# abhro/MonteCarloScattering.jl

Hardware: AMD Instinct MI355X
Metric: particle-scatter steps/sec + wall-time per iter, 10^6 particles, 1->8 MI355X (higher is better)
Workload: dtype f64

## Files before the change

### montecarloscattering.jl_amd/csrc/mcs_api.hip

```cpp
#include "mcs_launch.h"
#include "mcs_hip_owned.h"
#include "mcs_ctx_view.h"
#include "../../include/mcs_ic.h"

#include <cmath>
#include <cstdio>
#include <cstdlib>
#include <cstring>
#include <string>
#include <vector>
#include <chrono>
#include <cstdarg>
#include <memory>
#include <utility>

#define MCS_MEV_ERG_ 1.602176634e-6
namespace {
thread_local std::string g_err;

int fail(const std::string& msg) { g_err = msg; return 1; }
#define HIPCHK(expr)                                                                         \
  do {                                                                                       \
    hipError_t e_ = (expr);                                                                  \
    if (e_ != hipSuccess) return fail(std::string(#expr) + ": " + hipGetErrorString(e_));    \
  } while (0)
#define MCS_ENTER_AS(c, who) do { if (!(c)) return fail(std::string(who) + ": null context"); HIPCHK(hipSetDevice((c)->device)); } while (0)
#define MCS_ENTER(c) MCS_ENTER_AS(c, __func__)

std::string format(const char* f, ...) {
  char b[320];
  va_list ap; va_start(ap, f); std::vsnprintf(b, sizeof b, f, ap); va_end(ap);
  return b;
}
template <class B> int reserve(B& b, long long n) {
  const hipError_t e = b.reserve(n);
  return e == hipSuccess ? 0 : fail(std::string(B::alloc_name()) + ": " + hipGetErrorString(e));
}

constexpr double* DevPop::*kPopF64[8] = {&DevPop::weight, &DevPop::ptot_pf, &DevPop::pb_pf, &DevPop::x_PT_cm,
                                         &DevPop::xn_per, &DevPop::prp_x_cm, &DevPop::acctime_sec, &DevPop::phi_rad};
constexpr double* mcs_soa::*kSoaF64[8] = {&mcs_soa::weight, &mcs_soa::ptot_pf, &mcs_soa::pb_pf, &mcs_soa::x_PT_cm,
                                          &mcs_soa::xn_per, &mcs_soa::prp_x_cm, &mcs_soa::acctime_sec, &mcs_soa::phi_rad};
DevPop pop_view(const PopBuf& b, long long first = 0) {
  DevPop d{};
  for (int i = 0; i < 8; ++i) d.*kPopF64[i] = b.f[i] + first;
  d.meta = b.meta + first;
  return d;
}

struct StragBuf : BufGroup<StragBuf> {
  DevBuf<double> d[2];
  long long cap() const { return d[1].cap() / MCS_STRAG_WORDS; }
  hipError_t grow(long long n) { return reserve_all({n * MCS_STRAG_WORDS, n * MCS_STRAG_WORDS}, d[0], d[1]); }
};
struct FusedBuf : BufGroup<FusedBuf> {
  PinnedBuf<KArgs> h_args; PinnedBuf<PcutDev> h_pd; DevBuf<KArgs> d_args; DevBuf<PcutDev> d_pd;
  long long cap() const { return d_args.cap(); }
  hipError_t grow(long long n) { return reserve_all({n, n + 1, n, n + 1}, h_args, h_pd, d_args, d_pd); }
};

enum Ctr { CTR_WORK, CTR_SAVED, CTR_SCAN, CTR_EXPORT, CTR_MISMATCH, CTR_COUNT = 8 };
enum PipeCtr { PC_WORK, PC_SAVED, PC_SCAN, PC_EXPORT, PC_RES_WORK = PC_EXPORT + 2, PC_RES_SAVED, PC_LATE_WORK, PC_LATE_SAVED, PC_LATE_SCAN, PC_COUNT = 16 };
void set_counters(KArgs& a, unsigned long long* ctr, int work, int saved, int exported) {
  a.work_counter = ctr + work; a.n_saved = ctr + saved; a.strag_count = ctr + exported;
}
}

struct mcs_ctx {
  mcs_params P;
  mcs_layout L;
  int device = 0;
  Stream own_stream;
  hipStream_t stream = nullptr;
  DevBuf<double> d_tab;
  DevBuf<double> d_cuts;
  DevTables tb{};
  std::vector<double> h_inj_fracs, h_pcuts, h_ux;
  DevBuf<double> own_T; DevBuf<unsigned long long> own_I;
  double* d_T = nullptr; unsigned long long* d_I = nullptr;
  PopBuf cur, sav, spare;
  DevBuf<uint8_t> d_lsave;
  long long n = 0;
  long long n_saved_last = 0;
  long long n_run_last = 0;
  long long idx_first = 0, idx_stride = 1;
  const long long* idx_gidx = nullptr;
  bool debug_finals = false;
  int retro_cap = MCS_RETRO_CAP;
  int tail_rounds_last = 0;
  StragBuf strag;
  int64_t opt[MCS_OPT_COUNT] = {};
  long long o(int key) const { return opt[key]; }
  FinalsBuf fin; ScanScratch scan;
  DevBuf<double> d_tally_rep;
  long long rep_n = 0;
  bool rep_dirty = false;
  DevBuf<unsigned long long> d_counters;
  DevBuf<double> d_stage;
  PinnedBuf<KArgs> h_args_pin; DevBuf<KArgs> d_args;
  PinnedBuf<unsigned long long> h_back;
  int i_iter = 1, i_ion = 1;
  double aa = 1, zzq = MCS_QCGS, m = MCS_MP, mc = MCS_MP * MCS_C, pmax_cutoff = 0, density = 1, ewf = 1;
  bool have_grid = false, have_cuts = false;
  bool all_parallel = false;
  int kernel_last = -1;
  FusedBuf fused;
  std::vector<Event> f_ev;
  Stream pp_s2; Event pp_reset;
  Stream pp_s1m, pp_s2m; bool pp_masks_tried = false;
  PopBuf pp_sav2; DevBuf<uint8_t> pp_lsave2; ScanScratch pp_scan;
  DevBuf<unsigned long long> pp_dpc; PinnedBuf<unsigned long long> pp_hpc;
  PinnedBuf<KArgs> pp_hargs; DevBuf<KArgs> pp_dargs; DevBuf<PcutDev> pp_dpdl; PinnedBuf<PcutDev> pp_hpdl;
  int pp_waits_last = 0;
  DevBuf<double> d_ctab, d_cout, d_cscratch; DevBuf<unsigned long long> d_cdiag;
  bool have_cout_dndp = false, have_cout_thermo = false;
  DevBuf<double> d_c2d; bool have_c2d = false;
  int blocks = 0, threads = 256;
  Event ev0, ev1;
  Event acc_ev;
  double last_ms = 0.0;
  int n_cu = 256;
};

namespace {

int ensure_capacity(mcs_ctx* c, long long n) {
  if (n > c->cur.cap() || n > c->sav.cap()) {
    const long long cap = grow_cap(n);
    if (c->n > 0 && c->cur.cap() < cap) {
      PopBuf nb;
      if (reserve(nb, cap)) return 1;
      for (int i = 0; i < 8; ++i) HIPCHK(hipMemcpyAsync(nb.f[i], c->cur.f[i], (size_t)c->n * sizeof(double), hipMemcpyDeviceToDevice, c->stream));
      HIPCHK(hipMemcpyAsync(nb.meta, c->cur.meta, (size_t)c->n * sizeof(uint32_t), hipMemcpyDeviceToDevice, c->stream));
      HIPCHK(hipStreamSynchronize(c->stream));
      c->cur = std::move(nb);
    } else if (reserve(c->cur, cap)) return 1;
    if (reserve(c->sav, cap)) return 1;
  }
  if (n > c->d_lsave.cap() && reserve(c->d_lsave, grow_cap(n))) return 1;
  if (c->debug_finals && n > c->fin.cap() && reserve(c->fin, grow_cap(n))) return 1;
  if (n > c->scan.cap() && reserve(c->scan, grow_cap(n))) return 1;
  return 0;
}

int fill(mcs_ctx* c, long long off, long long n, double v) {
  HIPCHK(mcs_launch_fill(c->d_T + off, n, v, c->stream));
  return 0;
}

int upload_soa(mcs_ctx* c, const PopBuf& b, long long n, const mcs_soa* h) {
  for (int i = 0; i < 8; ++i) HIPCHK(hipMemcpyAsync(b.f[i], h->*kSoaF64[i], (size_t)n * sizeof(double), hipMemcpyHostToDevice, c->stream));
  std::vector<uint32_t> meta((size_t)n);
  for (long long k = 0; k < n; ++k) meta[k] = mcs_pack_meta((int)h->grid[k], (int)h->tcut[k], h->downstream[k] != 0, h->inj[k] != 0);
  HIPCHK(hipMemcpyAsync(b.meta, meta.data(), (size_t)n * sizeof(uint32_t), hipMemcpyHostToDevice, c->stream));
  HIPCHK(hipStreamSynchronize(c->stream));
  return 0;
}
int download_soa(mcs_ctx* c, const PopBuf& b, long long n, mcs_soa* h) {
  for (int i = 0; i < 8; ++i) HIPCHK(hipMemcpyAsync(h->*kSoaF64[i], b.f[i], (size_t)n * sizeof(double), hipMemcpyDeviceToHost, c->stream));
// ... 517 lines not shown
  HIPCHK(mcs_launch_compact(c->d_lsave, n, c->scan.bcounts, c->scan.boffs, c->d_counters + CTR_SCAN, c->scan.src, c->stream));
  HIPCHK(hipMemcpyAsync(c->h_back + CTR_SAVED, c->d_counters + CTR_SAVED, 3 * sizeof(unsigned long long), hipMemcpyDeviceToHost, c->stream));
  HIPCHK(hipStreamSynchronize(c->stream));
  const unsigned long long ns[2] = {c->h_back[CTR_SAVED], c->h_back[CTR_SCAN]};
  if (ws && c->h_back[CTR_EXPORT] != 0) {
    return fail(format("mcs_run_pcut: a bounded wait of the wave-specialised kernel ran out (the launch is incomplete; code 0x%llx)", (unsigned long long)c->h_back[CTR_EXPORT]));
  }
  if (budget == 0) {
    float ms = 0.f;
    HIPCHK(hipEventElapsedTime(&ms, c->ev0, c->ev1));
    ms_total = ms;
  }
  c->last_ms = ms_total;
  c->n_saved_last = (long long)ns[0];
  c->n_run_last = n; c->idx_first = i_prt_offset; c->idx_stride = i_prt_stride; c->idx_gidx = (const long long*)dev_gidx;
  if (ns[0] != ns[1]) return fail("mcs_run_pcut: the kernel's n_saved counter and the count of l_save flags differ");
  if (n_saved) *n_saved = (int64_t)ns[0];
  return 0;
}
int mcs_run_pcut_strided(mcs_ctx* c, int i_pcut, int64_t i_prt_offset, int64_t i_prt_stride, int64_t* n_saved) {
  return run_pcut_impl(c, i_pcut, i_prt_offset, i_prt_stride, nullptr, n_saved);
}
int mcs_run_pcut(mcs_ctx* c, int i_pcut, int64_t i_prt_offset, int64_t* n_saved) { return run_pcut_impl(c, i_pcut, i_prt_offset, 1, nullptr, n_saved); }
int mcs_run_pcut_indexed(mcs_ctx* c, int i_pcut, const int64_t* dev_gidx, int64_t* n_saved) {
  MCS_ENTER(c);
  if (!dev_gidx && c->n > 0) return fail("mcs_run_pcut_indexed: null index list");
  return run_pcut_impl(c, i_pcut, 0, 1, dev_gidx, n_saved);
}

struct PcutOut { int64_t *n_use, *n_saved, *i_mult; double* kernel_ms; int64_t* strag; };

static int species_loop_open(mcs_ctx* c, const char* who, int i_pcut_first, int i_pcut_last, const int64_t* n_target, const PcutOut& o, long long* cap_n) {
  const std::string w = std::string(who) + ": ";
  if (!c->have_grid || !c->have_cuts) return fail(w + "grid/cuts not set");
  if (i_pcut_first < 1 || i_pcut_last > c->tb.n_pcuts || i_pcut_last < i_pcut_first) return fail(w + "pcut range");
  if (!n_target || !o.n_use || !o.n_saved || !o.i_mult) return fail(w + "null argument");
  if (c->o(MCS_OPT_TAIL_BUDGET) > 0 || c->blocks > 0) return fail(w + "not with sliced launches or an explicit launch geometry");
  *cap_n = c->n;
  for (int k = 0; k <= i_pcut_last - i_pcut_first; ++k) { if (n_target[k] < 1) return fail(w + "n_target < 1"); if (n_target[k] > *cap_n) *cap_n = n_target[k]; }
  return ensure_capacity(c, *cap_n) || reserve(c->spare, grow_cap(*cap_n));
}

int mcs_run_pcuts_fused(mcs_ctx* c, int i_pcut_first, int i_pcut_last, const int64_t* n_target, int64_t* n_use_out, int64_t* n_saved_out,
                        int64_t* i_mult_out, double* kernel_ms_out) {
  MCS_ENTER(c);
  const PcutOut o{n_use_out, n_saved_out, i_mult_out, kernel_ms_out, nullptr};
  const int npc = i_pcut_last - i_pcut_first + 1;
  long long cap_n = 0;
  if (species_loop_open(c, "mcs_run_pcuts_fused", i_pcut_first, i_pcut_last, n_target, o, &cap_n)) return 1;
  if (npc > c->fused.cap()) {
    HIPCHK(hipStreamSynchronize(c->stream));
    if (reserve(c->fused, npc)) return 1;
  }
  while ((int)c->f_ev.size() < 2 * npc) { Event e; HIPCHK(e.create()); c->f_ev.push_back(std::move(e)); }
  const DevPop pop[2] = {pop_view(c->cur), pop_view(c->spare)}, sav = pop_view(c->sav);
  for (int k = 0; k < npc; ++k) {
    KArgs& a = c->fused.h_args[k];
    fill_kargs(c, a, i_pcut_first + k, 0, 0, 1, nullptr, 0);
    a.in = pop[k & 1]; a.sv = sav;
    a.n_dev = &c->fused.d_pd[k].n_use;
  }
  const K1Plan k1 = k1_plan(c, cap_n, false, false);
  const int blocks = persistent_grid(cap_n, k1.threads, (long long)c->n_cu * k1.per_cu);
  std::memset(c->fused.h_pd, 0, sizeof(PcutDev) * (size_t)(npc + 1));
  c->fused.h_pd[0].n_use = c->n;
  HIPCHK(hipMemcpyAsync(c->fused.d_args, c->fused.h_args, sizeof(KArgs) * (size_t)npc, hipMemcpyHostToDevice, c->stream));
  HIPCHK(hipMemcpyAsync(c->fused.d_pd, c->fused.h_pd, sizeof(PcutDev) * (size_t)(npc + 1), hipMemcpyHostToDevice, c->stream));
  HIPCHK(hipMemsetAsync(c->d_counters, 0, CTR_COUNT * sizeof(unsigned long long), c->stream));
  const int split_blocks = (int)std::min<long long>((cap_n + 255) / 256, (long long)c->n_cu * 16);
  for (int k = 0; k < npc; ++k) {
    HIPCHK(hipMemsetAsync(c->d_lsave, 0, (size_t)cap_n, c->stream));
    HIPCHK(hipEventRecord(c->f_ev[2 * k], c->stream));
    HIPCHK(mcs_launch_transport(c->fused.d_args + k, k1.kernel, blocks, k1.threads, c->stream));
    HIPCHK(hipEventRecord(c->f_ev[2 * k + 1], c->stream));
    HIPCHK(mcs_launch_finalize_split_dev(c->d_lsave, cap_n, c->scan.bcounts, c->scan.boffs, c->d_counters + CTR_SCAN, c->scan.src, c->fused.d_pd + k, c->fused.d_pd + k + 1,
                                         c->d_counters, (long long)n_target[k], c->d_counters + CTR_MISMATCH, sav, pop[(k + 1) & 1], split_blocks, c->stream));
  }
  c->rep_dirty = true;
  HIPCHK(hipMemcpyAsync(c->fused.h_pd, c->fused.d_pd, sizeof(PcutDev) * (size_t)(npc + 1), hipMemcpyDeviceToHost, c->stream));
  HIPCHK(hipMemcpyAsync(c->h_back + CTR_EXPORT, c->d_counters + CTR_EXPORT, 2 * sizeof(unsigned long long), hipMemcpyDeviceToHost, c->stream));
  HIPCHK(hipStreamSynchronize(c->stream));
  if (c->h_back[CTR_MISMATCH] != 0) return fail("mcs_run_pcuts_fused: the kernel's n_saved counter and the count of l_save flags differ");
  if (is_ws(k1.kernel) && c->h_back[CTR_EXPORT] != 0) return fail("mcs_run_pcuts_fused: a bounded wait of the wave-specialised kernel ran out (a launch is incomplete)");
  double ms_sum = 0.0;
  for (int k = 0; k < npc; ++k) {
    o.n_use[k] = c->fused.h_pd[k].n_use; o.n_saved[k] = c->fused.h_pd[k].n_saved; o.i_mult[k] = c->fused.h_pd[k].i_mult;
    float ms = 0.f;
    HIPCHK(hipEventElapsedTime(&ms, c->f_ev[2 * k], c->f_ev[2 * k + 1]));
    if (o.kernel_ms) o.kernel_ms[k] = ms;
    ms_sum += ms;
  }
  int n_split = 0; while (n_split < npc && c->fused.h_pd[n_split].n_saved > 0) ++n_split;
  if (n_split & 1) std::swap(c->cur, c->spare);
  c->n = c->fused.h_pd[n_split].n_use;
  c->n_run_last = -1; c->n_saved_last = 0;
  c->last_ms = ms_sum; c->tail_rounds_last = npc;
  c->kernel_last = k1.kernel;
  return 0;
}

static int pipelined_pcuts(mcs_ctx* c, const K1Plan& k1, int i_pcut_first, int npc, long long cap_n, const int64_t* n_target,
                           int64_t long_draws, int64_t long_imult_max, const PcutOut& o) {
  unsigned long long* const pc = c->pp_dpc;
  const bool masked = c->pp_s1m && c->pp_s2m;
  hipStream_t s1 = c->stream;
  hipStream_t const s2 = masked ? c->pp_s2m : c->pp_s2;
  hipStream_t const s_alone = masked ? c->stream : c->pp_s2;
  const int side_max = 64;
  const int threads = k1.threads;
  const long long full = (long long)c->n_cu * k1.per_cu;
  const DevPop savb[2] = {pop_view(c->sav), pop_view(c->pp_sav2)};
  uint8_t* lsv[2] = {c->d_lsave, c->pp_lsave2};
  long long nA = c->n, nL = 0;
  long long Bk = long_draws;
  bool side_pending = false;
  int side_blocks = 0;
  long long n1_prev = 0, sofar_prev = 0;
  c->pp_waits_last = 0;
  c->tail_rounds_last = 0;
  c->last_ms = 0.0;
  const bool dbg_pipe = std::getenv("MCS_PIPE_DEBUG") != nullptr;
  for (int k = 0; k < npc; ++k) { o.n_use[k] = 0; o.n_saved[k] = 0; o.i_mult[k] = 1; if (o.kernel_ms) o.kernel_ms[k] = 0.0; if (o.strag) { o.strag[2 * k] = 0; o.strag[2 * k + 1] = 0; } }
  HIPCHK(hipMemsetAsync(pc, 0, PC_COUNT * sizeof(unsigned long long), s1));
  if (nA > 0) HIPCHK(hipMemsetAsync(lsv[0], 0, (size_t)nA, s1));
  auto launch_resume = [&](int i_pcut, int q, long long n_pop, long long n_x, hipStream_t st, bool alone) -> int {
    KArgs& a = c->pp_hargs[1];
    fill_kargs(c, a, i_pcut, n_pop, 0, 1, nullptr, 0);
    a.in = pop_view(c->cur); a.sv = savb[q]; a.l_save = lsv[q];
    set_counters(a, pc, PC_RES_WORK, PC_RES_SAVED, PC_EXPORT + (q ^ 1)); a.strag_out = c->strag.d[q ^ 1];
// ... 498 lines not shown
```

### montecarloscattering.jl_amd/csrc/mcs_launch.h

```cpp
#pragma once
#include "mcs_device.h"

extern "C" {
int mcs_transport_max_entries(void);
hipError_t mcs_launch_transport(const KArgs* a_dev, int kernel, int blocks, int threads, hipStream_t st);
int mcs_transport_ws_threads(void);
hipError_t mcs_launch_finalize_split_dev(const uint8_t* l_save, long long cap_n, unsigned int* block_counts, unsigned long long* block_offsets,
                                         unsigned long long* scan_total, long long* src, PcutDev* pd, PcutDev* pd_next, unsigned long long* counters,
                                         long long n_target, unsigned long long* err, DevPop sv, DevPop out, int split_blocks, hipStream_t st);
hipError_t mcs_launch_compact(const uint8_t* l_save, long long n, unsigned int* block_counts, unsigned long long* block_offsets,
                              unsigned long long* total_dev, long long* src, hipStream_t st);
hipError_t mcs_launch_split(DevPop sv, DevPop out, const long long* src, long long n_new, long long i_mult, hipStream_t st);
hipError_t mcs_launch_compact_match(const uint8_t* l_save, long long n, unsigned int* block_counts, unsigned long long* block_offsets,
                                    unsigned long long* total_dev, long long* src, unsigned int match, hipStream_t st);
hipError_t mcs_launch_late_split(const uint8_t* l_save, long long n, unsigned int* block_counts, unsigned long long* block_offsets,
                                 unsigned long long* total_dev, long long* src, PcutDev* pd, long long i_mult, long long n_main_next, DevPop sv,
                                 DevPop out_at_main_end, int split_blocks, hipStream_t st);
hipError_t mcs_launch_saved_export(DevPop sv, const long long* src, long long n_saved, long long cap, long long first,
                                   long long stride, const long long* gin, long long* gidx, double* f64, uint32_t* meta,
                                   hipStream_t st);
hipError_t mcs_launch_split_import(DevPop out, const double* f64, const uint32_t* meta, long long cap, long long i_mult,
                                   long long first, long long stride, long long n_local, hipStream_t st);
hipError_t mcs_launch_init_pop(DevPop out, const double* ptot_in, const double* weight_in, long long n, long long j_offset,
                               long long j_stride, long long n_total, unsigned long long key, double m, double u, double x_start,
                               int i_grid_start, int relativistic, int fast_push, double xn_per_fine, double x_grid_stop,
                               int n_bins, const double* bin_ptot, const double* bin_weight, const long long* bin_start,
                               hipStream_t st);
hipError_t mcs_launch_fill(double* p, long long n, double v, hipStream_t st);
hipError_t mcs_launch_fold_replicas(double* dst, double* rep, long long n, int n_rep, hipStream_t st);
hipError_t mcs_launch_accumulate_tallies(double* dT, double* sT, unsigned long long* dI, unsigned long long* sI, long long a_lo,
                                         long long a_n, long long b_lo, long long b_n, long long i_lo, long long i_n, hipStream_t st);
hipError_t mcs_launch_copy(double* dst, const double* src, long long n, hipStream_t st);
hipError_t mcs_launch_eval(int fn, long long n, const double* a, const double* b, double* out, hipStream_t st);
hipError_t mcs_launch_eval_hot(int fn, long long n, const double* a, const double* b, double* out, hipStream_t st);
hipError_t mcs_launch_eval_scatter(const KArgs* a_dev, int form, long long n, const double* in, double* out, hipStream_t st);
hipError_t mcs_launch_dndp_cr(const mcs_params* P, const double* psd, const double* gam_sf, const double* ux, const double* tabs,
                              double rest_energy, double n0, double gam0, double* out_dndp, unsigned long long* diag, hipStream_t st);
hipError_t mcs_launch_dndp_2d(const mcs_params* P, const double* psd, const double* therm_sf, const unsigned long long* num_crossings, const double* tabs,
                              double rest_energy, double n0, int therm_from_hist, double gam_x, double beta_x, double* scratch, double* ef, hipStream_t st);
hipError_t mcs_launch_photon_ic(const double* ef, const double* p_edge, const double* field, int n_grid, int NM, int NT, int j_max, int n_nu, int n_photon,
                                double log_min_rm, double bins_per_dec, double mc_e, double beam_area, double* out, hipStream_t st);
hipError_t mcs_launch_photon_pion(const double* dndp_pf, const double* p_edge, const double* target, int n_grid, int NM, int n_photon,
                                  double log_emin_erg, double bins_per_dec, double mc, double aa, double scaling, int i_data, double* out, hipStream_t st);
hipError_t mcs_launch_photon_synch(const double* dndp_pf, const double* p_edge, const double* btot, int n_grid, int NM, int n_photon,
                                   double log_emin_erg, double bins_per_dec, double mc, double* out, hipStream_t st);
hipError_t mcs_launch_thermo(const mcs_params* P, const double* psd, const double* therm_pf, const unsigned long long* num_crossings,
                             const double* gam_sf, const double* ux, const double* tabs, double rest_energy, double mc, double n0,
                             int therm_from_hist, double* scratch, double* out3, hipStream_t st);
}
```

### montecarloscattering.jl_amd/csrc/mcs_population.hip

```cpp
#include "mcs_device.h"
#include "mcs_launch.h"
#include "../../include/mcs_math.h"

#pragma clang fp contract(off)

namespace {
constexpr double TWOPI_ = 6.283185307179586;
constexpr double CC_ = MCS_C;

__device__ __forceinline__ void philox_block(uint32_t c0, uint32_t c1, uint32_t c2, uint32_t c3, uint32_t k0,
                                             uint32_t k1, uint32_t& o0, uint32_t& o1, uint32_t& o2, uint32_t& o3) {
#pragma unroll
  for (int r = 0; r < 10; ++r) {
    const uint32_t hi0 = __umulhi(0xD2511F53u, c0), lo0 = 0xD2511F53u * c0;
    const uint32_t hi1 = __umulhi(0xCD9E8D57u, c2), lo1 = 0xCD9E8D57u * c2;
    const uint32_t n0 = hi1 ^ c1 ^ k0, n2 = hi0 ^ c3 ^ k1;
    c0 = n0; c1 = lo1; c2 = n2; c3 = lo0;
    k0 += 0x9E3779B9u; k1 += 0xBB67AE85u;
  }
  o0 = c0; o1 = c1; o2 = c2; o3 = c3;
}
__device__ __forceinline__ double philox_uniform(unsigned long long key, uint32_t stream, unsigned long long j) {
  const unsigned long long blk = j >> 1;
  uint32_t o0, o1, o2, o3;
// ... 26 lines not shown
  __shared__ unsigned long long sh[1024];
  __shared__ unsigned long long carry;
  if (threadIdx.x == 0) carry = 0;
  __syncthreads();
  for (long long c0 = 0; c0 < nb; c0 += 1024) {
    const long long i = c0 + threadIdx.x;
    const unsigned long long v = i < nb ? counts[i] : 0ull;
    sh[threadIdx.x] = v;
    __syncthreads();
    for (int off = 1; off < 1024; off <<= 1) {
      unsigned long long t = threadIdx.x >= (unsigned)off ? sh[threadIdx.x - off] : 0ull;
      __syncthreads();
      sh[threadIdx.x] += t;
      __syncthreads();
    }
    if (i < nb) offsets[i] = carry + sh[threadIdx.x] - v;
    __syncthreads();
    if (threadIdx.x == 1023) carry += sh[1023];
    __syncthreads();
  }
  if (threadIdx.x == 0) *total = carry;
}

extern "C" __global__ void __launch_bounds__(256)
mcs_k_compact_index(const uint8_t* __restrict__ l_save, long long n, const unsigned long long* __restrict__ offsets,
                    long long* __restrict__ src, unsigned int match) {
  __shared__ unsigned int wcount[4][4];
  const long long base = (long long)blockIdx.x * 1024;
  const int wave = threadIdx.x >> 6, lane = threadIdx.x & 63;
  bool f[4];
  unsigned long long m[4];
#pragma unroll
  for (int r = 0; r < 4; ++r) {
    const long long i = base + r * 256 + threadIdx.x;
    f[r] = i < n && l_save[i] == match;
    m[r] = __ballot(f[r]);
    if (lane == 0) wcount[r][wave] = (unsigned int)__popcll(m[r]);
  }
  __syncthreads();
  unsigned long long run = offsets[blockIdx.x];
#pragma unroll
  for (int r = 0; r < 4; ++r) {
    unsigned long long before = run;
    for (int w = 0; w < wave; ++w) before += wcount[r][w];
    if (f[r]) {
      const unsigned long long rank = before + (unsigned long long)__popcll(m[r] & ((1ull << lane) - 1ull));
      src[rank] = base + r * 256 + threadIdx.x;
    }
    run += wcount[r][0] + wcount[r][1] + wcount[r][2] + wcount[r][3];
  }
}

extern "C" __global__ void __launch_bounds__(256)
mcs_k_count_saved_dev(const uint8_t* __restrict__ l_save, const PcutDev* __restrict__ pd, unsigned int* __restrict__ block_counts) {
  __shared__ unsigned int wsum[4];
  const long long n = pd->n_use;
  const long long base = (long long)blockIdx.x * 1024;
  unsigned int c = 0;
  if (base < n) {
#pragma unroll
    for (int r = 0; r < 4; ++r) {
      const long long i = base + r * 256 + threadIdx.x;
      const bool f = i < n && l_save[i] == 1;
      c += (unsigned int)__popcll(__ballot(f));
    }
  }
  if ((threadIdx.x & 63) == 0) wsum[threadIdx.x >> 6] = c;
  __syncthreads();
  if (threadIdx.x == 0) block_counts[blockIdx.x] = wsum[0] + wsum[1] + wsum[2] + wsum[3];
}
extern "C" __global__ void __launch_bounds__(256)
mcs_k_compact_index_dev(const uint8_t* __restrict__ l_save, const PcutDev* __restrict__ pd, const unsigned long long* __restrict__ offsets,
                        long long* __restrict__ src) {
  __shared__ unsigned int wcount[4][4];
  const long long n = pd->n_use;
  const long long base = (long long)blockIdx.x * 1024;
  if (base >= n) return;
  const int wave = threadIdx.x >> 6, lane = threadIdx.x & 63;
  bool f[4];
  unsigned long long m[4];
#pragma unroll
  for (int r = 0; r < 4; ++r) {
    const long long i = base + r * 256 + threadIdx.x;
    f[r] = i < n && l_save[i] == 1;
    m[r] = __ballot(f[r]);
    if (lane == 0) wcount[r][wave] = (unsigned int)__popcll(m[r]);
  }
  __syncthreads();
  unsigned long long run = offsets[blockIdx.x];
#pragma unroll
  for (int r = 0; r < 4; ++r) {
    unsigned long long before = run;
    for (int w = 0; w < wave; ++w) before += wcount[r][w];
    if (f[r]) {
      const unsigned long long rank = before + (unsigned long long)__popcll(m[r] & ((1ull << lane) - 1ull));
      src[rank] = base + r * 256 + threadIdx.x;
    }
    run += wcount[r][0] + wcount[r][1] + wcount[r][2] + wcount[r][3];
  }
}
extern "C" __global__ void mcs_k_pcut_decide(PcutDev* __restrict__ pd, PcutDev* __restrict__ pd_next, const unsigned long long* __restrict__ scan_total,
                                             unsigned long long* __restrict__ counters , long long n_target,
                                             unsigned long long* __restrict__ err) {
  if (threadIdx.x != 0 || blockIdx.x != 0) return;
  const long long ns = (long long)*scan_total;
  if ((unsigned long long)ns != counters[1]) atomicAdd(err, 1ull);
  const long long im = ns > 0 ? (n_target / ns > 1 ? n_target / ns : 1) : 1;
  pd->n_saved = ns; pd->i_mult = im; pd->n_new = ns * im;
  if (pd_next) pd_next->n_use = ns * im;
  counters[0] = 0ull; counters[1] = 0ull;
}
extern "C" __global__ void mcs_k_late_decide(PcutDev* __restrict__ pd, const unsigned long long* __restrict__ scan_total, long long i_mult,
                                             long long n_main_next) {
  if (threadIdx.x != 0 || blockIdx.x != 0) return;
  const long long ns = (long long)*scan_total;
  pd->n_saved = ns; pd->i_mult = i_mult; pd->n_new = ns * i_mult; pd->n_use = n_main_next + ns * i_mult;
}
extern "C" __global__ void __launch_bounds__(256)
mcs_k_split_dev(DevPop sv, DevPop out, const long long* __restrict__ src, const PcutDev* __restrict__ pd) {
  const long long n_new = pd->n_new, i_mult = pd->i_mult;
  for (long long o = (long long)blockIdx.x * blockDim.x + threadIdx.x; o < n_new; o += (long long)gridDim.x * blockDim.x) {
    const long long j = src[o / i_mult];
    out.weight[o] = sv.weight[j] / (double)i_mult;
    out.ptot_pf[o] = sv.ptot_pf[j];
    out.pb_pf[o] = sv.pb_pf[j];
    out.x_PT_cm[o] = sv.x_PT_cm[j];
    out.xn_per[o] = sv.xn_per[j];
    out.prp_x_cm[o] = sv.prp_x_cm[j];
    out.acctime_sec[o] = sv.acctime_sec[j];
    out.phi_rad[o] = sv.phi_rad[j];
    out.meta[o] = sv.meta[j];
  }
}

extern "C" __global__ void __launch_bounds__(256)
mcs_k_split(DevPop sv, DevPop out, const long long* __restrict__ src, long long n_new, long long i_mult) {
  const long long o = (long long)blockIdx.x * blockDim.x + threadIdx.x;
  if (o >= n_new) return;
  const long long j = src[o / i_mult];
  out.weight[o] = sv.weight[j] / (double)i_mult;
  out.ptot_pf[o] = sv.ptot_pf[j];
  out.pb_pf[o] = sv.pb_pf[j];
  out.x_PT_cm[o] = sv.x_PT_cm[j];
  out.xn_per[o] = sv.xn_per[j];
  out.prp_x_cm[o] = sv.prp_x_cm[j];
  out.acctime_sec[o] = sv.acctime_sec[j];
  out.phi_rad[o] = sv.phi_rad[j];
  out.meta[o] = sv.meta[j];
}

extern "C" __global__ void __launch_bounds__(256)
mcs_k_saved_export(DevPop sv, const long long* __restrict__ src, long long n_saved, long long cap, long long first,
                   long long stride, const long long* __restrict__ gin, long long* __restrict__ gidx, double* __restrict__ f64,
                   uint32_t* __restrict__ meta) {
  const long long r = (long long)blockIdx.x * blockDim.x + threadIdx.x;
  if (r >= n_saved) return;
  const long long j = src[r];
  gidx[r] = gin ? gin[j] : first + j * stride;
  if (!f64) return;
  f64[r] = sv.weight[j];
  f64[cap + r] = sv.ptot_pf[j];
  f64[2 * cap + r] = sv.pb_pf[j];
  f64[3 * cap + r] = sv.x_PT_cm[j];
  f64[4 * cap + r] = sv.xn_per[j];
  f64[5 * cap + r] = sv.prp_x_cm[j];
  f64[6 * cap + r] = sv.acctime_sec[j];
  f64[7 * cap + r] = sv.phi_rad[j];
  meta[r] = sv.meta[j];
}
extern "C" __global__ void __launch_bounds__(256)
mcs_k_split_import(DevPop out, const double* __restrict__ f64, const uint32_t* __restrict__ meta, long long cap,
                   long long i_mult, long long first, long long stride, long long n_local) {
  const long long k = (long long)blockIdx.x * blockDim.x + threadIdx.x;
  if (k >= n_local) return;
  const long long j = (first + k * stride) / i_mult;
  out.weight[k] = f64[j] / (double)i_mult;
  out.ptot_pf[k] = f64[cap + j];
  out.pb_pf[k] = f64[2 * cap + j];
  out.x_PT_cm[k] = f64[3 * cap + j];
  out.xn_per[k] = f64[4 * cap + j];
  out.prp_x_cm[k] = f64[5 * cap + j];
  out.acctime_sec[k] = f64[6 * cap + j];
  out.phi_rad[k] = f64[7 * cap + j];
  out.meta[k] = meta[j];
// ... 49 lines not shown

extern "C" __global__ void mcs_k_fill_f64(double* p, long long n, double v) {
  for (long long i = (long long)blockIdx.x * blockDim.x + threadIdx.x; i < n; i += (long long)gridDim.x * blockDim.x) p[i] = v;
}
extern "C" __global__ void mcs_k_copy_f64(double* dst, const double* src, long long n) {
  for (long long i = (long long)blockIdx.x * blockDim.x + threadIdx.x; i < n; i += (long long)gridDim.x * blockDim.x) dst[i] = src[i];
}

extern "C" __global__ void mcs_k_eval_fn(int fn, long long n, const double* a, const double* b, double* out) {
  const long long i = (long long)blockIdx.x * blockDim.x + threadIdx.x;
  if (i >= n) return;
  double r = __builtin_nan("");
  switch (fn) {
    case MCS_FN_SIN: r = mcsm::sin(a[i]); break;
    case MCS_FN_COS: r = mcsm::cos(a[i]); break;
    case MCS_FN_ASIN: r = mcsm::asin(a[i]); break;
    case MCS_FN_ACOS: r = mcsm::acos(a[i]); break;
    case MCS_FN_ATAN2: r = mcsm::atan2(a[i], b[i]); break;
    case MCS_FN_LOG10: r = mcsm::log10(a[i]); break;
    case MCS_FN_MOD2PI: r = mcsm::mod2pi(a[i]); break;
    case MCS_FN_SQRT: r = __builtin_sqrt(a[i]); break;
    case MCS_FN_DIV: r = a[i] / b[i]; break;
    case MCS_FN_HYPOT1: r = mcsm::hypot1(a[i]); break;
    case MCS_FN_UNIFORM: r = philox_uniform((unsigned long long)a[i], 0u, (unsigned long long)b[i]); break;
    default: break;
  }
  out[i] = r;
}

extern "C" {

hipError_t mcs_launch_compact_match(const uint8_t* l_save, long long n, unsigned int* block_counts, unsigned long long* block_offsets,
                                    unsigned long long* total_dev, long long* src, unsigned int match, hipStream_t st) {
  const long long nb = (n + 1023) / 1024;
  if (nb == 0) return hipMemsetAsync(total_dev, 0, sizeof(unsigned long long), st);
  hipLaunchKernelGGL(mcs_k_count_saved, dim3((unsigned)nb), dim3(256), 0, st, l_save, n, block_counts, match);
  hipLaunchKernelGGL(mcs_k_scan_blocks, dim3(1), dim3(1024), 0, st, block_counts, nb, block_offsets, total_dev);
  hipLaunchKernelGGL(mcs_k_compact_index, dim3((unsigned)nb), dim3(256), 0, st, l_save, n, block_offsets, src, match);
  return hipGetLastError();
}
hipError_t mcs_launch_compact(const uint8_t* l_save, long long n, unsigned int* block_counts, unsigned long long* block_offsets,
                              unsigned long long* total_dev, long long* src, hipStream_t st) {
  return mcs_launch_compact_match(l_save, n, block_counts, block_offsets, total_dev, src, 1u, st);
}
hipError_t mcs_launch_late_split(const uint8_t* l_save, long long n, unsigned int* block_counts, unsigned long long* block_offsets,
                                 unsigned long long* total_dev, long long* src, PcutDev* pd, long long i_mult, long long n_main_next, DevPop sv,
                                 DevPop out_at_main_end, int split_blocks, hipStream_t st) {
  hipError_t e = mcs_launch_compact_match(l_save, n, block_counts, block_offsets, total_dev, src, 5u, st);
  if (e != hipSuccess) return e;
  hipLaunchKernelGGL(mcs_k_late_decide, dim3(1), dim3(64), 0, st, pd, total_dev, i_mult, n_main_next);
  hipLaunchKernelGGL(mcs_k_split_dev, dim3((unsigned)split_blocks), dim3(256), 0, st, sv, out_at_main_end, src, pd);
  return hipGetLastError();
}
hipError_t mcs_launch_finalize_split_dev(const uint8_t* l_save, long long cap_n, unsigned int* block_counts, unsigned long long* block_offsets,
                                         unsigned long long* scan_total, long long* src, PcutDev* pd, PcutDev* pd_next, unsigned long long* counters,
                                         long long n_target, unsigned long long* err, DevPop sv, DevPop out, int split_blocks, hipStream_t st) {
  const long long nb = (cap_n + 1023) / 1024;
  hipLaunchKernelGGL(mcs_k_count_saved_dev, dim3((unsigned)nb), dim3(256), 0, st, l_save, pd, block_counts);
  hipLaunchKernelGGL(mcs_k_scan_blocks, dim3(1), dim3(1024), 0, st, block_counts, nb, block_offsets, scan_total);
  hipLaunchKernelGGL(mcs_k_compact_index_dev, dim3((unsigned)nb), dim3(256), 0, st, l_save, pd, block_offsets, src);
  hipLaunchKernelGGL(mcs_k_pcut_decide, dim3(1), dim3(64), 0, st, pd, pd_next, scan_total, counters, n_target, err);
  hipLaunchKernelGGL(mcs_k_split_dev, dim3((unsigned)split_blocks), dim3(256), 0, st, sv, out, src, pd);
  return hipGetLastError();
}
hipError_t mcs_launch_split(DevPop sv, DevPop out, const long long* src, long long n_new, long long i_mult, hipStream_t st) {
  if (n_new > 0)
    hipLaunchKernelGGL(mcs_k_split, dim3((unsigned)((n_new + 255) / 256)), dim3(256), 0, st, sv, out, src, n_new, i_mult);
  return hipGetLastError();
}
hipError_t mcs_launch_saved_export(DevPop sv, const long long* src, long long n_saved, long long cap, long long first,
                                   long long stride, const long long* gin, long long* gidx, double* f64, uint32_t* meta,
                                   hipStream_t st) {
  if (n_saved > 0)
    hipLaunchKernelGGL(mcs_k_saved_export, dim3((unsigned)((n_saved + 255) / 256)), dim3(256), 0, st, sv, src, n_saved, cap,
                       first, stride, gin, gidx, f64, meta);
  return hipGetLastError();
}
hipError_t mcs_launch_split_import(DevPop out, const double* f64, const uint32_t* meta, long long cap, long long i_mult,
                                   long long first, long long stride, long long n_local, hipStream_t st) {
  if (n_local > 0)
    hipLaunchKernelGGL(mcs_k_split_import, dim3((unsigned)((n_local + 255) / 256)), dim3(256), 0, st, out, f64, meta, cap,
                       i_mult, first, stride, n_local);
  return hipGetLastError();
}

hipError_t mcs_launch_init_pop(DevPop out, const double* ptot_in, const double* weight_in, long long n, long long j_offset,
                               long long j_stride, long long n_total, unsigned long long key, double m, double u, double x_start,
                               int i_grid_start, int relativistic, int fast_push, double xn_per_fine, double x_grid_stop,
                               int n_bins, const double* bin_ptot, const double* bin_weight, const long long* bin_start,
                               hipStream_t st) {
  if (n <= 0) return hipSuccess;
  hipLaunchKernelGGL(mcs_k_init_pop, dim3((unsigned)((n + 255) / 256)), dim3(256), 0, st, out, ptot_in, weight_in, n,
                     j_offset, j_stride, n_total, key, m, u, x_start, i_grid_start, relativistic, fast_push, xn_per_fine, x_grid_stop,
                     n_bins, bin_ptot, bin_weight, bin_start);
  return hipGetLastError();
}

hipError_t mcs_launch_fill(double* p, long long n, double v, hipStream_t st) {
  if (n <= 0) return hipSuccess;
  long long blocks = (n + 255) / 256;
  if (blocks > 4096) blocks = 4096;
  hipLaunchKernelGGL(mcs_k_fill_f64, dim3((unsigned)blocks), dim3(256), 0, st, p, n, v);
  return hipGetLastError();
}
hipError_t mcs_launch_copy(double* dst, const double* src, long long n, hipStream_t st) {
  if (n <= 0) return hipSuccess;
  long long blocks = (n + 255) / 256;
  if (blocks > 4096) blocks = 4096;
  hipLaunchKernelGGL(mcs_k_copy_f64, dim3((unsigned)blocks), dim3(256), 0, st, dst, src, n);
  return hipGetLastError();
}
hipError_t mcs_launch_eval(int fn, long long n, const double* a, const double* b, double* out, hipStream_t st) {
  if (fn < 0 || fn > MCS_FN_UNIFORM) return hipErrorInvalidValue;
  if (n <= 0) return hipSuccess;
  hipLaunchKernelGGL(mcs_k_eval_fn, dim3((unsigned)((n + 255) / 256)), dim3(256), 0, st, fn, n, a, b, out);
// ... 44 lines not shown
```

Baseline: 44.69 billion.

## Fuse pcut finalize into count+last-block scan kernel and select-based split

Replaces the five-kernel finalize chain (count, scan, compact index, decide, split) with two kernels. The first counts flags per block and uses an atomic ticket so the last block does the scan and the pcut decision. The second locates each output's source particle by binary-searching the block offsets and ranking within the ballot masks, so the src index array is never built. The per-pcut memset of l_save is replaced by double-buffered flag arrays that the finalize kernel clears in place, which removes launches and memsets per pcut. In exchange it adds a serial single-block scan, repeated mask reconstruction in the split kernel, and reliance on memory fences for the last-block pattern.

```diff
diff --git a/montecarloscattering.jl_amd/csrc/mcs_api.hip b/montecarloscattering.jl_amd/csrc/mcs_api.hip
--- a/montecarloscattering.jl_amd/csrc/mcs_api.hip
+++ b/montecarloscattering.jl_amd/csrc/mcs_api.hip
@@ -59,7 +59,7 @@
   hipError_t grow(long long n) { return reserve_all({n, n + 1, n, n + 1}, h_args, h_pd, d_args, d_pd); }
 };
 
-enum Ctr { CTR_WORK, CTR_SAVED, CTR_SCAN, CTR_EXPORT, CTR_MISMATCH, CTR_COUNT = 8 };
+enum Ctr { CTR_WORK, CTR_SAVED, CTR_SCAN, CTR_EXPORT, CTR_MISMATCH, CTR_TICKET, CTR_COUNT = 8 };
 enum PipeCtr { PC_WORK, PC_SAVED, PC_SCAN, PC_EXPORT, PC_RES_WORK = PC_EXPORT + 2, PC_RES_SAVED, PC_LATE_WORK, PC_LATE_SAVED, PC_LATE_SCAN, PC_COUNT = 16 };
 void set_counters(KArgs& a, unsigned long long* ctr, int work, int saved, int exported) {
   a.work_counter = ctr + work; a.n_saved = ctr + saved; a.strag_count = ctr + exported;
@@ -104,7 +104,7 @@
   bool have_grid = false, have_cuts = false;
   bool all_parallel = false;
   int kernel_last = -1;
-  FusedBuf fused;
+  FusedBuf fused; DevBuf<uint8_t> f_lsave2;
   std::vector<Event> f_ev;
   Stream pp_s2; Event pp_reset;
   Stream pp_s1m, pp_s2m; bool pp_masks_tried = false;
@@ -728,12 +728,14 @@
     HIPCHK(hipStreamSynchronize(c->stream));
     if (reserve(c->fused, npc)) return 1;
   }
+  if (cap_n > c->f_lsave2.cap() && reserve(c->f_lsave2, grow_cap(cap_n))) return 1;
   while ((int)c->f_ev.size() < 2 * npc) { Event e; HIPCHK(e.create()); c->f_ev.push_back(std::move(e)); }
   const DevPop pop[2] = {pop_view(c->cur), pop_view(c->spare)}, sav = pop_view(c->sav);
+  uint8_t* const lsv[2] = {c->d_lsave, c->f_lsave2};
   for (int k = 0; k < npc; ++k) {
     KArgs& a = c->fused.h_args[k];
     fill_kargs(c, a, i_pcut_first + k, 0, 0, 1, nullptr, 0);
-    a.in = pop[k & 1]; a.sv = sav;
+    a.in = pop[k & 1]; a.sv = sav; a.l_save = lsv[k & 1];
     a.n_dev = &c->fused.d_pd[k].n_use;
   }
   const K1Plan k1 = k1_plan(c, cap_n, false, false);
@@ -744,13 +746,13 @@
   HIPCHK(hipMemcpyAsync(c->fused.d_pd, c->fused.h_pd, sizeof(PcutDev) * (size_t)(npc + 1), hipMemcpyHostToDevice, c->stream));
   HIPCHK(hipMemsetAsync(c->d_counters, 0, CTR_COUNT * sizeof(unsigned long long), c->stream));
   const int split_blocks = (int)std::min<long long>((cap_n + 255) / 256, (long long)c->n_cu * 16);
+  HIPCHK(hipMemsetAsync(lsv[0], 0, (size_t)cap_n, c->stream));
   for (int k = 0; k < npc; ++k) {
-    HIPCHK(hipMemsetAsync(c->d_lsave, 0, (size_t)cap_n, c->stream));
     HIPCHK(hipEventRecord(c->f_ev[2 * k], c->stream));
     HIPCHK(mcs_launch_transport(c->fused.d_args + k, k1.kernel, blocks, k1.threads, c->stream));
     HIPCHK(hipEventRecord(c->f_ev[2 * k + 1], c->stream));
-    HIPCHK(mcs_launch_finalize_split_dev(c->d_lsave, cap_n, c->scan.bcounts, c->scan.boffs, c->d_counters + CTR_SCAN, c->scan.src, c->fused.d_pd + k, c->fused.d_pd + k + 1,
-                                         c->d_counters, (long long)n_target[k], c->d_counters + CTR_MISMATCH, sav, pop[(k + 1) & 1], split_blocks, c->stream));
+    HIPCHK(mcs_launch_finalize_split_dev(lsv[k & 1], lsv[(k + 1) & 1], cap_n, c->scan.bcounts, c->scan.boffs, c->fused.d_pd + k, c->fused.d_pd + k + 1, c->d_counters,
+                                         c->d_counters + CTR_TICKET, (long long)n_target[k], c->d_counters + CTR_MISMATCH, sav, pop[(k + 1) & 1], split_blocks, c->stream));
   }
   c->rep_dirty = true;
   HIPCHK(hipMemcpyAsync(c->fused.h_pd, c->fused.d_pd, sizeof(PcutDev) * (size_t)(npc + 1), hipMemcpyDeviceToHost, c->stream));
diff --git a/montecarloscattering.jl_amd/csrc/mcs_launch.h b/montecarloscattering.jl_amd/csrc/mcs_launch.h
--- a/montecarloscattering.jl_amd/csrc/mcs_launch.h
+++ b/montecarloscattering.jl_amd/csrc/mcs_launch.h
@@ -5,9 +5,10 @@
 int mcs_transport_max_entries(void);
 hipError_t mcs_launch_transport(const KArgs* a_dev, int kernel, int blocks, int threads, hipStream_t st);
 int mcs_transport_ws_threads(void);
-hipError_t mcs_launch_finalize_split_dev(const uint8_t* l_save, long long cap_n, unsigned int* block_counts, unsigned long long* block_offsets,
-                                         unsigned long long* scan_total, long long* src, PcutDev* pd, PcutDev* pd_next, unsigned long long* counters,
-                                         long long n_target, unsigned long long* err, DevPop sv, DevPop out, int split_blocks, hipStream_t st);
+hipError_t mcs_launch_finalize_split_dev(const uint8_t* l_save, uint8_t* l_clear, long long cap_n, unsigned int* block_counts,
+                                         unsigned long long* block_offsets, PcutDev* pd, PcutDev* pd_next, unsigned long long* counters,
+                                         unsigned long long* ticket, long long n_target, unsigned long long* err, DevPop sv, DevPop out,
+                                         int split_blocks, hipStream_t st);
 hipError_t mcs_launch_compact(const uint8_t* l_save, long long n, unsigned int* block_counts, unsigned long long* block_offsets,
                               unsigned long long* total_dev, long long* src, hipStream_t st);
 hipError_t mcs_launch_split(DevPop sv, DevPop out, const long long* src, long long n_new, long long i_mult, hipStream_t st);
diff --git a/montecarloscattering.jl_amd/csrc/mcs_population.hip b/montecarloscattering.jl_amd/csrc/mcs_population.hip
--- a/montecarloscattering.jl_amd/csrc/mcs_population.hip
+++ b/montecarloscattering.jl_amd/csrc/mcs_population.hip
@@ -102,63 +102,79 @@
 }
 
 extern "C" __global__ void __launch_bounds__(256)
-mcs_k_count_saved_dev(const uint8_t* __restrict__ l_save, const PcutDev* __restrict__ pd, unsigned int* __restrict__ block_counts) {
+mcs_k_finalize_dev(const uint8_t* __restrict__ l_save, uint8_t* __restrict__ l_clear, long long n_clear, PcutDev* __restrict__ pd,
+                   PcutDev* __restrict__ pd_next, unsigned int* block_counts, unsigned long long* __restrict__ offsets,
+                   unsigned long long* __restrict__ counters , unsigned long long* ticket, long long n_target,
+                   unsigned long long* __restrict__ err) {
   __shared__ unsigned int wsum[4];
+  __shared__ int last;
   const long long n = pd->n_use;
   const long long base = (long long)blockIdx.x * 1024;
+  const int wave = threadIdx.x >> 6, lane = threadIdx.x & 63;
   unsigned int c = 0;
   if (base < n) {
+    uint8_t st[4];
 #pragma unroll
     for (int r = 0; r < 4; ++r) {
       const long long i = base + r * 256 + threadIdx.x;
-      const bool f = i < n && l_save[i] == 1;
-      c += (unsigned int)__popcll(__ballot(f));
-    }
-  }
-  if ((threadIdx.x & 63) == 0) wsum[threadIdx.x >> 6] = c;
+      st[r] = l_save[i < n ? i : n - 1];
+    }
+#pragma unroll
+    for (int r = 0; r < 4; ++r) c += (unsigned int)__popcll(__ballot(base + r * 256 + threadIdx.x < n && st[r] == 1));
+  }
+  if (lane == 0) wsum[wave] = c;
   __syncthreads();
-  if (threadIdx.x == 0) block_counts[blockIdx.x] = wsum[0] + wsum[1] + wsum[2] + wsum[3];
-}
-extern "C" __global__ void __launch_bounds__(256)
-mcs_k_compact_index_dev(const uint8_t* __restrict__ l_save, const PcutDev* __restrict__ pd, const unsigned long long* __restrict__ offsets,
-                        long long* __restrict__ src) {
-  __shared__ unsigned int wcount[4][4];
-  const long long n = pd->n_use;
-  const long long base = (long long)blockIdx.x * 1024;
-  if (base >= n) return;
-  const int wave = threadIdx.x >> 6, lane = threadIdx.x & 63;
-  bool f[4];
-  unsigned long long m[4];
-#pragma unroll
-  for (int r = 0; r < 4; ++r) {
-    const long long i = base + r * 256 + threadIdx.x;
-    f[r] = i < n && l_save[i] == 1;
-    m[r] = __ballot(f[r]);
-    if (lane == 0) wcount[r][wave] = (unsigned int)__popcll(m[r]);
+  if (threadIdx.x == 0) {
+    __hip_atomic_store(block_counts + blockIdx.x, wsum[0] + wsum[1] + wsum[2] + wsum[3], __ATOMIC_RELAXED, __HIP_MEMORY_SCOPE_AGENT);
+    __builtin_amdgcn_fence(__ATOMIC_RELEASE, "agent");
+    asm volatile("s_waitcnt vmcnt(0)" ::: "memory");
+    last = atomicAdd(ticket, 1ull) == (unsigned long long)gridDim.x - 1ull;
+  }
+  {
+    const long long i = base + 4 * (long long)threadIdx.x;
+    if (i + 4 <= n_clear) *reinterpret_cast<uint32_t*>(l_clear + i) = 0u;
+    else for (long long t = i; t < n_clear; ++t) l_clear[t] = 0;
   }
   __syncthreads();
-  unsigned long long run = offsets[blockIdx.x];
-#pragma unroll
-  for (int r = 0; r < 4; ++r) {
-    unsigned long long before = run;
-    for (int w = 0; w < wave; ++w) before += wcount[r][w];
-    if (f[r]) {
-      const unsigned long long rank = before + (unsigned long long)__popcll(m[r] & ((1ull << lane) - 1ull));
-      src[rank] = base + r * 256 + threadIdx.x;
-    }
-    run += wcount[r][0] + wcount[r][1] + wcount[r][2] + wcount[r][3];
-  }
-}
-extern "C" __global__ void mcs_k_pcut_decide(PcutDev* __restrict__ pd, PcutDev* __restrict__ pd_next, const unsigned long long* __restrict__ scan_total,
-                                             unsigned long long* __restrict__ counters , long long n_target,
-                                             unsigned long long* __restrict__ err) {
-  if (threadIdx.x != 0 || blockIdx.x != 0) return;
-  const long long ns = (long long)*scan_total;
+  if (!last) return;
+  __builtin_amdgcn_fence(__ATOMIC_ACQUIRE, "agent");
+
+  const long long nb = (n + 1023) / 1024;
+  unsigned long long carry = 0;
+  for (long long c0 = 0; c0 < nb; c0 += 1024) {
+    const long long i0 = c0 + 4 * (long long)threadIdx.x;
+    unsigned int v[4], s = 0;
+#pragma unroll
+    for (int t = 0; t < 4; ++t) {
+      v[t] = i0 + t < nb ? __hip_atomic_load(block_counts + i0 + t, __ATOMIC_RELAXED, __HIP_MEMORY_SCOPE_AGENT) : 0u;
+      s += v[t];
+    }
+    unsigned int incl = s;
+#pragma unroll
+    for (int off = 1; off < 64; off <<= 1) {
+      const unsigned int up = __shfl_up(incl, off);
+      if (lane >= off) incl += up;
+    }
+    __syncthreads();
+    if (lane == 63) wsum[wave] = incl;
+    __syncthreads();
+    unsigned long long run = carry + (incl - s);
+    for (int w = 0; w < wave; ++w) run += wsum[w];
+#pragma unroll
+    for (int t = 0; t < 4; ++t) {
+      if (i0 + t < nb) offsets[i0 + t] = run;
+      run += v[t];
+    }
+    carry += (unsigned long long)wsum[0] + wsum[1] + wsum[2] + wsum[3];
+  }
+  if (threadIdx.x != 0) return;
+  const long long ns = (long long)carry;
   if ((unsigned long long)ns != counters[1]) atomicAdd(err, 1ull);
   const long long im = ns > 0 ? (n_target / ns > 1 ? n_target / ns : 1) : 1;
   pd->n_saved = ns; pd->i_mult = im; pd->n_new = ns * im;
   if (pd_next) pd_next->n_use = ns * im;
   counters[0] = 0ull; counters[1] = 0ull;
+  *ticket = 0ull;
 }
 extern "C" __global__ void mcs_k_late_decide(PcutDev* __restrict__ pd, const unsigned long long* __restrict__ scan_total, long long i_mult,
                                              long long n_main_next) {
@@ -180,6 +196,79 @@
     out.acctime_sec[o] = sv.acctime_sec[j];
     out.phi_rad[o] = sv.phi_rad[j];
     out.meta[o] = sv.meta[j];
+  }
+}
+__device__ __forceinline__ long long mcs_find_block(const unsigned long long* __restrict__ offsets, long long nb, unsigned long long pos) {
+  long long lo = 0, hi = nb;
+  while (hi - lo > 1) { const long long mid = (lo + hi) >> 1; if (offsets[mid] <= pos) lo = mid; else hi = mid; }
+  return lo;
+}
+extern "C" __global__ void __launch_bounds__(256)
+mcs_k_split_select_dev(DevPop sv, DevPop out, const uint8_t* __restrict__ l_save, const unsigned long long* __restrict__ offsets,
+                       const PcutDev* __restrict__ pd) {
+  const long long n = pd->n_use, n_new = pd->n_new, i_mult = pd->i_mult;
+  const long long nb = (n + 1023) / 1024;
+  const int lane = threadIdx.x & 63;
+  for (long long o0 = (long long)blockIdx.x * blockDim.x + (threadIdx.x & ~63u); o0 < n_new; o0 += (long long)gridDim.x * blockDim.x) {
+    const long long o = o0 + lane;
+    const bool active = o < n_new;
+    const long long pos = (active ? o : n_new - 1) / i_mult;
+    const long long pos0 = (long long)(((unsigned long long)__builtin_amdgcn_readfirstlane((unsigned int)((unsigned long long)pos >> 32)) << 32) |
+                                       __builtin_amdgcn_readfirstlane((unsigned int)pos));
+    long long b;
+    if (__all(pos == pos0)) b = mcs_find_block(offsets, nb, (unsigned long long)pos0);
+    else b = mcs_find_block(offsets, nb, (unsigned long long)pos);
+    const unsigned int rank = (unsigned int)((unsigned long long)pos - offsets[b]);
+    long long j = 0;
+    bool todo = true;
+    for (;;) {
+      const unsigned long long pending = __ballot(todo);
+      if (pending == 0ull) break;
+      const long long bb = __shfl(b, __ffsll((long long)pending) - 1);
+      const long long base = bb * 1024;
+      uint8_t st[16];
+#pragma unroll
+      for (int q = 0; q < 16; ++q) {
+        const long long i = base + q * 64 + lane;
+        st[q] = l_save[i < n ? i : n - 1];
+      }
+      unsigned long long m[16];
+#pragma unroll
+      for (int q = 0; q < 16; ++q) m[q] = __ballot(base + q * 64 + lane < n && st[q] == 1);
+      if (todo && b == bb) {
+        unsigned int r = rank;
+        unsigned long long mm = 0ull;
+        int qq = 0;
+        bool found = false;
+#pragma unroll
+        for (int q = 0; q < 16; ++q) {
+          const unsigned int c = (unsigned int)__popcll(m[q]);
+          if (!found) { if (r < c) { mm = m[q]; qq = q; found = true; } else r -= c; }
+        }
+        int bit = 0;
+#pragma unroll
+        for (int w = 32; w >= 1; w >>= 1) {
+          const unsigned int c = (unsigned int)__popcll(mm & ((1ull << w) - 1ull));
+          if (r >= c) { r -= c; mm >>= w; bit += w; }
+        }
+        j = found ? base + qq * 64 + bit : base;
+        todo = false;
+      }
+    }
+    if (active) {
+      const double weight = sv.weight[j], ptot_pf = sv.ptot_pf[j], pb_pf = sv.pb_pf[j], x_PT_cm = sv.x_PT_cm[j], xn_per = sv.xn_per[j],
+                   prp_x_cm = sv.prp_x_cm[j], acctime_sec = sv.acctime_sec[j], phi_rad = sv.phi_rad[j];
+      const uint32_t meta = sv.meta[j];
+      out.weight[o] = weight / (double)i_mult;
+      out.ptot_pf[o] = ptot_pf;
+      out.pb_pf[o] = pb_pf;
+      out.x_PT_cm[o] = x_PT_cm;
+      out.xn_per[o] = xn_per;
+      out.prp_x_cm[o] = prp_x_cm;
+      out.acctime_sec[o] = acctime_sec;
+      out.phi_rad[o] = phi_rad;
+      out.meta[o] = meta;
+    }
   }
 }
 
@@ -335,15 +424,14 @@
   hipLaunchKernelGGL(mcs_k_split_dev, dim3((unsigned)split_blocks), dim3(256), 0, st, sv, out_at_main_end, src, pd);
   return hipGetLastError();
 }
-hipError_t mcs_launch_finalize_split_dev(const uint8_t* l_save, long long cap_n, unsigned int* block_counts, unsigned long long* block_offsets,
-                                         unsigned long long* scan_total, long long* src, PcutDev* pd, PcutDev* pd_next, unsigned long long* counters,
-                                         long long n_target, unsigned long long* err, DevPop sv, DevPop out, int split_blocks, hipStream_t st) {
+hipError_t mcs_launch_finalize_split_dev(const uint8_t* l_save, uint8_t* l_clear, long long cap_n, unsigned int* block_counts,
+                                         unsigned long long* block_offsets, PcutDev* pd, PcutDev* pd_next, unsigned long long* counters,
+                                         unsigned long long* ticket, long long n_target, unsigned long long* err, DevPop sv, DevPop out,
+                                         int split_blocks, hipStream_t st) {
   const long long nb = (cap_n + 1023) / 1024;
-  hipLaunchKernelGGL(mcs_k_count_saved_dev, dim3((unsigned)nb), dim3(256), 0, st, l_save, pd, block_counts);
-  hipLaunchKernelGGL(mcs_k_scan_blocks, dim3(1), dim3(1024), 0, st, block_counts, nb, block_offsets, scan_total);
-  hipLaunchKernelGGL(mcs_k_compact_index_dev, dim3((unsigned)nb), dim3(256), 0, st, l_save, pd, block_offsets, src);
-  hipLaunchKernelGGL(mcs_k_pcut_decide, dim3(1), dim3(64), 0, st, pd, pd_next, scan_total, counters, n_target, err);
-  hipLaunchKernelGGL(mcs_k_split_dev, dim3((unsigned)split_blocks), dim3(256), 0, st, sv, out, src, pd);
+  hipLaunchKernelGGL(mcs_k_finalize_dev, dim3((unsigned)nb), dim3(256), 0, st, l_save, l_clear, cap_n, pd, pd_next, block_counts, block_offsets,
+                     counters, ticket, n_target, err);
+  hipLaunchKernelGGL(mcs_k_split_select_dev, dim3((unsigned)split_blocks), dim3(256), 0, st, sv, out, l_save, block_offsets, pd);
   return hipGetLastError();
 }
 hipError_t mcs_launch_split(DevPop sv, DevPop out, const long long* src, long long n_new, long long i_mult, hipStream_t st) {
```

Result: no change. 44.70 billion, median of 6 (+0.0%).
